# vilnik/incorporating-different-sources

Measured on AMD Instinct MI355X. Metric: rolling windows/sec, higher is better.
Workload: dtype f64

## Files before the change

### incorporating_different_sources_amd/csrc/posterior_wave_impl.h

```cpp
#pragma once
#include <utility>

#include "posterior_fused_impl.h"

namespace {

template <int NT_, bool LEAN_ = true>
struct WCfg {
    static constexpr int NT = NT_;
    static constexpr int KP = 16 * NT;
    static constexpr int NTILES = NT * (NT + 1) / 2;
    static constexpr int MLD = 17;
    static constexpr int OFF_M = 0;
    static constexpr int OFF_DG = OFF_M + NT * 16 * MLD;
    static constexpr int OFF_IDT = OFF_DG + 256;
    static constexpr int OFF_VEC = OFF_IDT + 256;
    static constexpr int LDS_DOUBLES = OFF_VEC + KP;
    static constexpr int LDS_BYTES = LDS_DOUBLES * 8;
    static constexpr int OFF_SUB = LDS_DOUBLES;
};
constexpr int WAVE_LDS_LIMIT = 64 * 1024;
__host__ __device__ inline int wave_idx_rows(int n_r, int m, bool conj) {
    const int r = (conj && m > n_r) ? m : n_r;
    return (r + 63) & ~63;
}
__host__ __device__ inline int wave_idx_bytes(int n_r, int m, bool conj) { return wave_idx_rows(n_r, m, conj) * 12; }

constexpr int wtile(int NT, int I, int J) { return I * NT - I * (I - 1) / 2 + (J - I); }

template <int I, int J>
__device__ __forceinline__ void wave_post_tile(double* P, int k, int fr, int fq, const d4& t) {
    const int gj = 16 * J + fr;
#pragma unroll
    for (int r = 0; r < 4; ++r) {
        const int gi = 16 * I + fq + 4 * r;
        if (gi < k && gj < k && (I < J || gi <= gj)) {
            tp_post_store(P + (long long)gi * k + gj, t[r]);
            if (I < J || gi < gj) tp_post_store(P + (long long)gj * k + gi, t[r]);
        }
    }
}

template <int NT, int NWV>
constexpr int w2_owner(int J) {
    const int p = NT - 1 - J, g = p / NWV, i = p % NWV;
    return (g & 1) ? NWV - 1 - i : i;
}
template <int NT, int NWV>
constexpr int w2_count(int WV) {
    int n = 0;
    for (int J = 0; J < NT; ++J)
        if (w2_owner<NT, NWV>(J) == WV) n += J + 1;
    return n;
}
template <int NT, int NWV>
constexpr int w2_max_tiles() {
    int m = 0;
    for (int w = 0; w < NWV; ++w) m = w2_count<NT, NWV>(w) > m ? w2_count<NT, NWV>(w) : m;
    return m;
}
template <int NT, int NWV>
constexpr int w2_slot(int I, int J) {
    const int wv = w2_owner<NT, NWV>(J);
    int n = 0;
    for (int i = 0; i < NT; ++i)
        for (int j = i; j < NT; ++j) {
            if (i == I && j == J) return n;
            if (w2_owner<NT, NWV>(j) == wv) ++n;
        }
    return -1;
}
template <int NT, int NWV>
constexpr bool w2_owns_from(int WV, int I) {
    for (int J = I; J < NT; ++J)
        if (w2_owner<NT, NWV>(J) == WV) return true;
    return false;
}
template <int NT>
constexpr bool w2_one_wave_is_whole() {
    for (int J = 0; J < NT; ++J) {
        if (w2_owner<NT, 1>(J) != 0) return false;
        for (int I = 0; I <= J; ++I)
            if (w2_slot<NT, 1>(I, J) != wtile(NT, I, J)) return false;
    }
    return w2_count<NT, 1>(0) == NT * (NT + 1) / 2;
}
template <int... N>
constexpr bool w2_one_wave_is_whole_all(std::integer_sequence<int, N...>) { return (w2_one_wave_is_whole<N + 1>() && ...); }
static_assert(w2_one_wave_is_whole_all(std::make_integer_sequence<int, 15>{}),
              "w2_owner<NT,1>(J) == 0, w2_slot<NT,1>(I,J) == wtile(NT,I,J), w2_count<NT,1>(0) == NT(NT+1)/2 for NT = 1..15");

constexpr bool wave_tile_in_agpr(int t) { return t < 32; }

template <int T>
__device__ __forceinline__ void wave_mfma_agpr(d4& c, double a, double b) {
    if constexpr (wave_tile_in_agpr(T)) asm volatile("s_nop 1\n\tv_mfma_f64_16x16x4_f64 %0, %1, %2, %0" : "+a"(c) : "v"(a), "v"(b));
    else asm volatile("s_nop 1\n\tv_mfma_f64_16x16x4_f64 %0, %1, %2, %0" : "+v"(c) : "v"(a), "v"(b));
}
template <int T>
__device__ __forceinline__ void wave_settle1(d4& c0) {
    if constexpr (wave_tile_in_agpr(T)) asm volatile("s_nop 15\n\ts_nop 7" : "+a"(c0));
    else asm volatile("s_nop 15\n\ts_nop 7" : "+v"(c0));
}
template <int T>
__device__ __forceinline__ void wave_pin1(d4& c0) {
    if constexpr (wave_tile_in_agpr(T)) asm volatile("" : "+a"(c0));
    else asm volatile("" : "+v"(c0));
}
__device__ __forceinline__ void wave_settle14(d4& c0, d4& c1, d4& c2, d4& c3, d4& c4, d4& c5, d4& c6, d4& c7, d4& c8, d4& c9,
                                              d4& c10, d4& c11, d4& c12, d4& c13) {
    asm volatile("s_nop 15\n\ts_nop 7" : "+a"(c0), "+a"(c1), "+a"(c2), "+a"(c3), "+a"(c4), "+a"(c5), "+a"(c6), "+a"(c7), "+a"(c8),
                 "+a"(c9), "+a"(c10), "+a"(c11), "+a"(c12), "+a"(c13));
}
template <int N>
__device__ __forceinline__ void wave_pin(d4 (&acc)[N]) {
    static_for<0, N>([&](auto tc) __attribute__((always_inline)) { wave_pin1<decltype(tc)::value>(acc[decltype(tc)::value]); });
}
template <bool GROUPED, int N>
__device__ __forceinline__ void wave_settle(d4 (&acc)[N]) {
    if constexpr (GROUPED) {
        static_for<0, (N + 13) / 14>([&](auto gc) __attribute__((always_inline)) {
            constexpr int b = 14 * decltype(gc)::value;
            if constexpr (b + 14 <= N && wave_tile_in_agpr(b + 13)) {
                wave_settle14(acc[b], acc[b + 1], acc[b + 2], acc[b + 3], acc[b + 4], acc[b + 5], acc[b + 6], acc[b + 7], acc[b + 8],
                              acc[b + 9], acc[b + 10], acc[b + 11], acc[b + 12], acc[b + 13]);
            } else {
                static_for<b, (b + 14 < N ? b + 14 : N)>([&](auto tc) __attribute__((always_inline)) {
                    wave_settle1<decltype(tc)::value>(acc[decltype(tc)::value]);
                });
            }
        });
    } else {
        wave_settle1<0>(acc[0]);
        static_for<1, N>([&](auto tc) __attribute__((always_inline)) { wave_pin1<decltype(tc)::value>(acc[decltype(tc)::value]); });
    }
}

struct WRows {
    const double* base;
    long long ld;
    const int* ridx;
    long long first;
    const double* sub_row;
    int count;
    int count0;
    int jump;
    bool off32 = false;
};

template <int NT, int NWV, int WV, bool HF, bool LEAN>
__device__ __forceinline__ void wave_gram(const WRows& src, const long long (&coff)[NT], int k, int lane,
                                          double (&shift)[NT], double (&w0v)[NT], bool ones, bool lazy_mask,
                                          d4 (&acc)[w2_count<NT, NWV>(WV)], const int* lds_rows, const double* lds_sub,
                                          double (&csum)[NT], double& usum) {
    constexpr int kI = NT - 1;
    const int fr = lane & 15, fq = lane >> 4;
    const int kc = k - 16 * kI;
    const bool cvl = fr < kc;
    const double border = HF ? ((ones && fr == kc + 1) ? 1.0 : 0.0) : ((fr == kc) ? 1.0 : 0.0);
    const int nks = (src.count + 3) >> 2;
    const bool has_sub = !HF && src.sub_row != nullptr;

    int row_pref = 0;
    double sub_pref = 0.0;
    auto prefetch = [&](int ks) __attribute__((always_inline)) {
        int r = 4 * ks + fq;
        r = r < src.count ? r : src.count - 1;
        row_pref = lds_rows[r];
        if (has_sub) sub_pref = lds_sub[r];
    };
    if constexpr (!LEAN) prefetch(0);
    const char* ub = (const char*)(LEAN ? src.base + src.first * src.ld : src.base);
    const unsigned ld8 = (unsigned)src.ld * 8u;
    unsigned c8[NT];
#pragma unroll
    for (int i = 0; i < NT; ++i) c8[i] = 8u * (unsigned)coff[i];
    auto load = [&](double (&v)[NT], double& sub, int ks) __attribute__((always_inline)) {
        int r = 4 * ks + fq;
        r = r < src.count ? r : src.count - 1;
        if (LEAN || src.off32) {
            unsigned row;
            if constexpr (LEAN) row = (unsigned)(r + (r >= src.count0 ? src.jump : 0));
            else row = (unsigned)row_pref;
            if constexpr (LEAN) {
                const unsigned r0 = __umul24(row, ld8) + c8[0];
#pragma unroll
                for (int i = 0; i < NT - 1; ++i) v[i] = *(const double*)(ub + (size_t)r0 + 128 * i);
                v[NT - 1] = *(const double*)(ub + (size_t)(__umul24(row, ld8) + c8[NT - 1]));
            } else {
                const unsigned ro = __umul24(row, ld8);
#pragma unroll
                for (int i = 0; i < NT; ++i) v[i] = *(const double*)(ub + (size_t)(ro + c8[i]));
            }
        } else {
            const double* p = src.base + (long long)row_pref * src.ld;
#pragma unroll
            for (int i = 0; i < NT; ++i) v[i] = p[coff[i]];
        }
        sub = 0.0;
        if constexpr (!LEAN) {
            if (has_sub) sub = sub_pref;
            prefetch(ks + 1);
        } else {
            if (has_sub) sub = src.sub_row[r];
        }
    };
    auto step = [&](double (&v)[NT], double sub, int ks, auto maskc) __attribute__((always_inline)) {
        constexpr bool MASK = decltype(maskc)::value != 0;
        if (HF) {
#pragma unroll
            for (int i = 0; i < NT; ++i) v[i] -= shift[i];
        } else if (has_sub) {
#pragma unroll
            for (int i = 0; i < NT; ++i) v[i] -= sub;
        }
        v[kI] = cvl ? v[kI] : border;
        if (MASK) {
            const bool rv = 4 * ks + fq < src.count;
#pragma unroll
            for (int i = 0; i < NT; ++i) v[i] = rv ? v[i] : 0.0;
        }
        if (HF) {
            double z = 0.0;
#pragma unroll
            for (int i = 0; i < NT; ++i) z = fma(v[i], w0v[i], z);
            z = rowgroup_sum16(z);
            if (!ones) {
#pragma unroll
                for (int i = 0; i < NT; ++i) csum[i] += v[i];
                usum += z;
            }
            if (fr == kc) v[kI] = z;
        }
        static_for<0, NT>([&](auto Ic) __attribute__((always_inline)) {
            constexpr int I = decltype(Ic)::value;
            static_for<I, NT>([&](auto Jc) __attribute__((always_inline)) {
                constexpr int J = decltype(Jc)::value;
                if constexpr (w2_owner<NT, NWV>(J) == WV) {
                    constexpr int t = w2_slot<NT, NWV>(I, J);
                    wave_mfma_agpr<t>(acc[t], v[I], v[J]);
                }
            });
        });
    };

    if (nks <= 0) return;
    double va[NT], vb[NT], vc[NT];
    double sa = 0.0, sb = 0.0, sc = 0.0;
    load(va, sa, 0);
    load(vb, sb, 1);
    if (HF && lazy_mask) {
        __builtin_amdgcn_sched_barrier(0);
#pragma unroll
        for (int i = 0; i < NT; ++i) {
            const bool cv = 16 * i + fr < k;
            shift[i] = cv ? shift[i] : 0.0;
            w0v[i] = cv ? w0v[i] : 0.0;
        }
    }
    wave_pin(acc);
    int ks = 0;
#pragma nounroll
    for (; 4 * (ks + 3) <= src.count; ks += 3) {
        load(vc, sc, ks + 2);
        step(va, sa, ks, ic<0>{});
        load(va, sa, ks + 3);
        step(vb, sb, ks + 1, ic<0>{});
        load(vb, sb, ks + 4);
        step(vc, sc, ks + 2, ic<0>{});
    }
    if (ks < nks) {
        if (ks + 2 < nks) load(vc, sc, ks + 2);
        step(va, sa, ks, ic<1>{});
        if (ks + 1 < nks) step(vb, sb, ks + 1, ic<1>{});
        if (ks + 2 < nks) step(vc, sc, ks + 2, ic<1>{});
    }
    wave_settle<NWV == 1>(acc);
}

__device__ __forceinline__ void wave_stage_rows(const WRows& src, int lane, int* li, double* lsb) {
    for (int i = lane; i < src.count; i += 64) {
        li[i] = src.ridx ? src.ridx[i] : (int)(src.first + i);
        if (src.sub_row) lsb[i] = src.sub_row[i];
    }
    __builtin_amdgcn_fence(__ATOMIC_RELEASE, "wavefront");
    __builtin_amdgcn_wave_barrier();
}

template <int NT, bool LEAN, int MODE>
__device__ __forceinline__ void wave_window_body(const tp_kargs_t& A, double* lds) {
    constexpr bool FULL = MODE == 2;
    constexpr bool POST = MODE >= 3;
    constexpr int PLAIN = POST ? MODE - 3 : MODE;
    using C = WCfg<NT, LEAN>;
    const int lane = threadIdx.x;
    const int fr = lane & 15, fq = lane >> 4;
    const int k = A.k;
    __builtin_assume(k >= 16 * (NT - 1));
    __builtin_assume(k <= 16 * NT - 1);
    constexpr int kI = NT - 1;
    const int kc = k - 16 * kI;
    const int NTB = (kc == 0) ? NT - 1 : NT;
    const bool colv = fr < kc;
    const long long per_xcd = (A.w_count + 7) >> 3;
    const long long wl = (long long)(blockIdx.x & 7) * per_xcd + (blockIdx.x >> 3);
    if ((long long)(blockIdx.x >> 3) >= per_xcd || wl >= A.w_count) return;
    const long long w = A.w_first + wl;
    const int tid0 = lane;
    (void)tid0;

    const int* cols = (!LEAN && A.col_idx) ? A.col_idx + w * k : nullptr;
    long long coff[NT];
    if (cols != nullptr) {
        int cidx[NT];
#pragma unroll
        for (int i = 0; i < NT; ++i) {
            const int c = 16 * i + fr;
            cidx[i] = cols[c < k ? c : k - 1];
        }
#pragma unroll
        for (int i = 0; i < NT; ++i) coff[i] = (long long)cidx[i];
    } else {
#pragma unroll
        for (int i = 0; i < NT; ++i) {
            const int c = 16 * i + fr;
            coff[i] = (long long)(c < k ? c : k - 1);
        }
    }
    double* idx_sub_lds = LEAN ? nullptr : lds + C::OFF_SUB;
    int* idx_rows_lds = LEAN ? nullptr : (int*)(lds + C::OFF_SUB + wave_idx_rows(A.n_r, A.m, A.strategy == 0));
    d4 acc[C::NTILES];
    static_for<0, C::NTILES>([&](auto tc) __attribute__((always_inline)) { acc[decltype(tc)::value] = d4{0.0, 0.0, 0.0, 0.0}; });
    wave_pin(acc);

#pragma unroll
    for (int i = 0; i < 4; ++i) {
        const int e = lane + 64 * i;
        lds[C::OFF_IDT + e] = ((e >> 4) == (e & 15)) ? 1.0 : 0.0;
    }

    double n0 = 0.0, cc = 0.0, q0 = 0.0;
    const bool conj = PLAIN == 0 ? true : PLAIN == 1 ? false : (A.strategy == 0);
    const int dbg = (FULL && A.dbg_S1 != nullptr && w == A.dbg_w) ? A.dbg_mode : 0;

    auto dump_matrix = [&]() __attribute__((always_inline)) {
        static_for<0, NT>([&](auto Ic) __attribute__((always_inline)) {
            constexpr int I = decltype(Ic)::value;
            static_for<I, NT>([&](auto Jc) __attribute__((always_inline)) {
                constexpr int J = decltype(Jc)::value;
                constexpr int t = wtile(NT, I, J);
                const int gj = 16 * J + fr;
#pragma unroll
                for (int r = 0; r < 4; ++r) {
                    const int gi = 16 * I + fq + 4 * r;
                    if (gi < k && gj < k) {
                        A.dbg_S1[(long long)gi * k + gj] = acc[t][r];
                        A.dbg_S1[(long long)gj * k + gi] = acc[t][r];
                    }
                    if (gi < k && gj == k) A.dbg_S1[(long long)k * k + gi] = acc[t][r];
                }
            });
        });
    };
    auto corner = [&]() __attribute__((always_inline)) {
        constexpr int t = wtile(NT, kI, kI);
        const int ln = __builtin_amdgcn_readfirstlane(16 * (kc & 3) + kc);
        const double x0 = readlane_d(acc[t][0], ln), x1 = readlane_d(acc[t][1], ln);
        const double x2 = readlane_d(acc[t][2], ln), x3 = readlane_d(acc[t][3], ln);
        const int rr = kc >> 2;
        return rr == 0 ? x0 : rr == 1 ? x1 : rr == 2 ? x2 : x3;
    };

    TP_MARK(0);
    if (conj && dbg != 2) {
        n0 = A.n0[w];
        WRows hs;
        hs.base = A.hf_panel; hs.ld = A.hf_ld;
        hs.ridx = (!LEAN && A.hf_row_idx) ? A.hf_row_idx + w * (long long)A.m : nullptr;
        hs.first = A.hf_start ? A.hf_start[w] : 0;
        hs.sub_row = nullptr;
        hs.count = A.hf_count ? A.hf_count[w] : A.m;
        hs.count0 = 0x7fffffff; hs.jump = 0;
        hs.off32 = (A.hf_off32 & 1) != 0;
        const bool ones = kc < 15;
        double shift[NT], w0v[NT], csum[NT];
        double usum = 0.0;
        {
            const long long row0 = hs.ridx ? (long long)hs.ridx[0] : hs.first;
            const double* p0 = hs.base + row0 * (long long)hs.ld;
#pragma unroll
            for (int i = 0; i < NT; ++i) {
                const int c = 16 * i + fr;
                const int cl = c < k ? c : k - 1;
                const double sv = p0[coff[i]];
                const double wv = A.w0[w * k + cl];
                shift[i] = sv;
                w0v[i] = wv;
                csum[i] = 0.0;
            }
        }
        TP_MARK(1);
        const int hf_rows_all = hs.count;
        if (!hs.ridx) { hs.first += 1; hs.count -= 1; }
        else { hs.ridx += 1; hs.count -= 1; }
        if constexpr (!LEAN) wave_stage_rows(hs, lane, idx_rows_lds, idx_sub_lds);
        wave_gram<NT, 1, 0, true, LEAN>(hs, coff, k, lane, shift, w0v, ones, true, acc, idx_rows_lds, idx_sub_lds, csum, usum);
        hs.count = hf_rows_all;
        TP_MARK(2);
        const double invm = 1.0 / (double)hs.count;
        double tj[NT];
        double cz = corner();
        if (ones) {
            static_for<0, NT>([&](auto Ic) __attribute__((always_inline)) {
                constexpr int I = decltype(Ic)::value;
                constexpr int t = wtile(NT, I, kI);
                if (fr == kc + 1) {
#pragma unroll
                    for (int r = 0; r < 4; ++r)
                        lds[C::OFF_VEC + 16 * I + fq + 4 * r] = (I < kI || fq + 4 * r <= kc) ? acc[t][r] : 0.0;
                }
            });
        } else {
#pragma unroll
            for (int i = 0; i < NT; ++i) {
                double sc_ = csum[i];
                sc_ += __shfl_xor(sc_, 16, 64);
                sc_ += __shfl_xor(sc_, 32, 64);
                if (fq == 0) lds[C::OFF_VEC + 16 * i + fr] = (16 * i + fr < k) ? sc_ : 0.0;
            }
            double su = usum;
            su += __shfl_xor(su, 16, 64);
            su += __shfl_xor(su, 32, 64);
            __builtin_amdgcn_fence(__ATOMIC_RELEASE, "wavefront");
            __builtin_amdgcn_wave_barrier();
            if (lane == 0) lds[C::OFF_VEC + k] = su;
        }
        __builtin_amdgcn_fence(__ATOMIC_RELEASE, "wavefront");
        __builtin_amdgcn_wave_barrier();
#pragma unroll
        for (int J = 0; J < NT; ++J) tj[J] = lds[C::OFF_VEC + 16 * J + fr];
        {
            const double tk = lds[C::OFF_VEC + k];
            cz = fma(-(tk * invm), tk, cz);
        }
        const double mm = (double)hs.count;
        const double sc = n0 * (mm / (mm - 1.0));
        q0 = sc * cz;
        const double a = n0 + k + 2;
        cc = (2 * n0) / (a + sqrt(a * a + 4 * n0 * q0));
        const double fcol = colv ? sc : ((fr == kc) ? cc * sc : 0.0);
        static_for<0, NT>([&](auto Ic) __attribute__((always_inline)) {
            constexpr int I = decltype(Ic)::value;
            double ti[4];
#pragma unroll
            for (int r = 0; r < 4; ++r) ti[r] = -(lds[C::OFF_VEC + 16 * I + fq + 4 * r] * invm);
            static_for<I, NT>([&](auto Jc) __attribute__((always_inline)) {
                constexpr int J = decltype(Jc)::value;
                constexpr int t = wtile(NT, I, J);
                d4 x = acc[t];
#pragma unroll
                for (int r = 0; r < 4; ++r) x[r] = fma(ti[r], tj[J], x[r]);
                if constexpr (J < kI) {
                    x *= sc;
                } else if constexpr (I < kI) {
                    x *= fcol;
                } else {
#pragma unroll
                    for (int r = 0; r < 4; ++r) x[r] *= (fq + 4 * r < kc) ? fcol : 0.0;
                }
                acc[t] = x;
                wave_pin1<t>(acc[t]);
            });
            __builtin_amdgcn_sched_barrier(0);
        });
        __builtin_amdgcn_wave_barrier();
        if (dbg == 1) { dump_matrix(); return; }
    }
    TP_MARK(3);
    {
        WRows ds;
        ds.base = A.panel; ds.ld = A.panel_ld;
        ds.ridx = (!LEAN && A.row_idx) ? A.row_idx + w * (long long)A.n_r : nullptr;
        ds.first = A.start ? A.start[w] : 0;
        ds.sub_row = A.rf_adj ? A.rf_adj + w * (long long)A.n_r : nullptr;
        ds.count = A.n_rows ? A.n_rows[w] : A.n_r;
        ds.count0 = 0x7fffffff; ds.jump = 0;
        ds.off32 = (A.panel_off32 & 1) != 0;
        double none[NT] = {};
        bool shared = false;
        const double* q = nullptr;
        if constexpr (LEAN) {
            constexpr int BLK = 16;
            const long long b0 = (ds.first + BLK - 1) / BLK, b1 = (ds.first + ds.count) / BLK;
            const int Lw = (int)(b1 - b0);
            const int li = Lw == A.winsum_L[0] ? 0 : Lw == A.winsum_L[1] ? 1 : Lw == A.winsum_L[2] ? 2 : Lw == A.winsum_L[3] ? 3 : -1;
            shared = A.winsum != nullptr && Lw > 0 && li >= 0;
            if (shared) {
                ds.count0 = (int)(BLK * b0 - ds.first);
                ds.jump = (int)(BLK * b1 - ds.first) - ds.count0;
                ds.count = ds.count0 + (int)(ds.first + ds.count - BLK * b1);
                q = A.winsum + ((long long)li * A.prefix_nblk + b0) * ((long long)C::NTILES * 256);
            }
        }
        TP_MARK(32);
        typedef double d2 __attribute__((ext_vector_type(2)));
        constexpr int GRP = 7, NG = (C::NTILES + GRP - 1) / GRP;
        const d2* pq = (const d2*)q + lane;
        d2 qa[GRP][2], qb[GRP][2];
        auto qload = [&](d2 (&v2)[GRP][2], auto gc) __attribute__((always_inline)) {
            constexpr int g = decltype(gc)::value;
            static_for<0, GRP>([&](auto ec) __attribute__((always_inline)) {
                constexpr int e = decltype(ec)::value;
                constexpr int t = g * GRP + e;
                if constexpr (t < C::NTILES) {
                    v2[e][0] = pq[(long long)t * 128];
                    v2[e][1] = pq[(long long)t * 128 + 64];
                }
            });
        };
        auto qadd = [&](d2 (&v2)[GRP][2], auto gc) __attribute__((always_inline)) {
            constexpr int g = decltype(gc)::value;
            static_for<0, GRP>([&](auto ec) __attribute__((always_inline)) {
                constexpr int e = decltype(ec)::value;
                constexpr int t = g * GRP + e;
                if constexpr (t < C::NTILES) {
                    d4 x = acc[t];
                    x[0] += v2[e][0][0]; x[1] += v2[e][0][1];
                    x[2] += v2[e][1][0]; x[3] += v2[e][1][1];
                    acc[t] = x;
                    wave_pin1<t>(acc[t]);
                }
            });
        };
        if constexpr (!LEAN) wave_stage_rows(ds, lane, idx_rows_lds, idx_sub_lds);
        double nosum = 0.0;
        wave_gram<NT, 1, 0, false, LEAN>(ds, coff, k, lane, none, none, false, false, acc, idx_rows_lds, idx_sub_lds, none, nosum);
        TP_MARK(33);
        if (LEAN && shared) {
            qload(qa, ic<0>{});
            static_for<0, NG>([&](auto gc) __attribute__((always_inline)) {
                constexpr int g = decltype(gc)::value;
                if constexpr (g + 1 < NG) {
                    if constexpr (g % 2 == 0) qload(qb, ic<g + 1>{}); else qload(qa, ic<g + 1>{});
                }
                __builtin_amdgcn_sched_barrier(0);
                if constexpr (g % 2 == 0) qadd(qa, gc); else qadd(qb, gc);
                __builtin_amdgcn_sched_barrier(0);
            });
        }
    }
    TP_MARK(34);
    static_for<0, NT>([&](auto Ic) __attribute__((always_inline)) {
        constexpr int I = decltype(Ic)::value;
        constexpr int t = wtile(NT, I, kI);
        if constexpr (I == kI) {
            d4 x = acc[t];
#pragma unroll
            for (int r = 0; r < 4; ++r) x[r] = (fq + 4 * r >= kc) ? 0.0 : x[r];
            acc[t] = x;
            wave_pin1<t>(acc[t]);
        }
    });
    __builtin_amdgcn_sched_barrier(0);
    if (dbg == 2) { dump_matrix(); return; }

    if (!conj) {
        static_for<0, NT>([&](auto Ic) __attribute__((always_inline)) {
            constexpr int I = decltype(Ic)::value;
            constexpr int t = wtile(NT, I, kI);
            if (fr == kc) {
#pragma unroll
                for (int r = 0; r < 4; ++r) lds[C::OFF_VEC + 16 * I + fq + 4 * r] = acc[t][r];
            }
        });
        __builtin_amdgcn_fence(__ATOMIC_RELEASE, "wavefront");
        __builtin_amdgcn_wave_barrier();
        const double invN = !FULL ? 1.0 / (double)A.N : A.center_rows == 2 ? 0.0
                          : 1.0 / (double)(A.center_rows ? (A.n_rows ? A.n_rows[w] : A.n_r) : A.N);
        const double sh_d = (FULL && A.shift) ? A.shift[2 * w] : 0.0;
        const double sh_e = (FULL && A.shift) ? A.shift[2 * w + 1] : 0.0;
        double tj[NT];
#pragma unroll
        for (int J = 0; J < NT; ++J) tj[J] = lds[C::OFF_VEC + 16 * J + fr];
        static_for<0, NT>([&](auto Ic) __attribute__((always_inline)) {
            constexpr int I = decltype(Ic)::value;
            double ti[4];
#pragma unroll
            for (int r = 0; r < 4; ++r) ti[r] = lds[C::OFF_VEC + 16 * I + fq + 4 * r];
            static_for<I, NT>([&](auto Jc) __attribute__((always_inline)) {
                constexpr int J = decltype(Jc)::value;
                constexpr int t = wtile(NT, I, J);
                d4 x = acc[t];
#pragma unroll
                for (int r = 0; r < 4; ++r) {
                    const bool on = (J < kI || colv) && (I < kI || fq + 4 * r < kc);
                    const double add = sh_e + ((I == J && fq + 4 * r == fr) ? sh_d : 0.0);
                    x[r] += on ? add - invN * (ti[r] * tj[J]) : 0.0;
                }
                acc[t] = x;
                wave_pin1<t>(acc[t]);
            });
            __builtin_amdgcn_sched_barrier(0);
        });
        __builtin_amdgcn_wave_barrier();
    }
    if (FULL && A.rhs != nullptr) {
        static_for<0, NT>([&](auto Ic) __attribute__((always_inline)) {
            constexpr int I = decltype(Ic)::value;
            constexpr int t = wtile(NT, I, kI);
            if (fr == kc) {
#pragma unroll
                for (int r = 0; r < 4; ++r) {
                    const int gi = 16 * I + fq + 4 * r;
                    const int gl = gi < k ? gi : k - 1;
                    const double x = A.rhs[w * k + gl];
                    acc[t][r] = (gi < k) ? x : 0.0;
                }
            }
            wave_pin1<t>(acc[t]);
        });
    }
    if (FULL && A.out_rhs != nullptr) {
        static_for<0, NT>([&](auto Ic) __attribute__((always_inline)) {
            constexpr int I = decltype(Ic)::value;
            constexpr int t = wtile(NT, I, kI);
            if (fr == kc) {
#pragma unroll
                for (int r = 0; r < 4; ++r) {
                    const int gi = 16 * I + fq + 4 * r;
                    if (gi < k) A.out_rhs[w * k + gi] = acc[t][r];
                }
            }
        });
    }
    if (dbg == 3) dump_matrix();
    if constexpr (POST) {
        double* P = tp_post_window(A, w);
        if (P != nullptr) {
            static_for<0, NT>([&](auto Ic) __attribute__((always_inline)) {
                constexpr int I = decltype(Ic)::value;
                static_for<I, NT>([&](auto Jc) __attribute__((always_inline)) {
                    constexpr int J = decltype(Jc)::value;
                    wave_post_tile<I, J>(P, k, fr, fq, acc[wtile(NT, I, J)]);
                });
            });
        }
    }

    TP_MARK(4);
    double badacc = 0.0;
    static_for<0, NT>([&](auto jc) __attribute__((always_inline)) {
        constexpr int j = decltype(jc)::value;
        if (j < NTB) {
            const int npiv = (k - 16 * j < 16) ? (k - 16 * j) : 16;
            constexpr int tjj = wtile(NT, j, j);
#pragma unroll
            for (int r = 0; r < 4; ++r) lds[C::OFF_DG + (fq + 4 * r) * 16 + fr] = acc[tjj][r];
            __builtin_amdgcn_fence(__ATOMIC_RELEASE, "wavefront");
            __builtin_amdgcn_wave_barrier();
            const int c16 = lane & 15;
            double a[16];
            const double* src = (lane < 16) ? (lds + C::OFF_DG) : (lds + C::OFF_IDT);
#pragma unroll
            for (int i = 0; i < 16; ++i) a[i] = src[i * 16 + c16];
            constexpr bool ALL16 = j < kI;
            double d0 = readlane_d(a[0], 0);
            double rinv = rsqrt_cubic(d0);
#pragma unroll
            for (int p = 0; p < 16; ++p) {
                if (ALL16 || p < npiv) {
                    a[p] *= rinv;
                    badacc = fma(0.0, rinv, badacc);
                    double rinv_next = 1.0;
                    if (p + 1 < 16) {
                        const double s1 = readlane_d(a[p], p + 1);
                        a[p + 1] = fma(-s1, a[p], a[p + 1]);
                        double dn = readlane_d(a[p + 1], p + 1);
                        if (!ALL16) dn = (p + 1 < npiv) ? dn : 1.0;
                        rinv_next = rsqrt_cubic(dn);
                    }
#pragma unroll
                    for (int i = p + 2; i < 16; ++i) {
                        const double sI = readlane_d(a[p], i);
                        a[i] = fma(-sI, a[p], a[i]);
                    }
                    rinv = rinv_next;
                    __builtin_amdgcn_sched_barrier(0);
                }
            }
            if (lane >= 16 && lane < 32) {
#pragma unroll
                for (int i = 0; i < 16; ++i) lds[C::OFF_M + (j * 16 + i) * C::MLD + c16] = (i < npiv) ? a[i] : 0.0;
            }
            __builtin_amdgcn_fence(__ATOMIC_RELEASE, "wavefront");
            __builtin_amdgcn_wave_barrier();
            double mop[4];
#pragma unroll
            for (int r = 0; r < 4; ++r) mop[r] = lds[C::OFF_M + (j * 16 + fr) * C::MLD + 4 * r + fq];
            static_for<j, NT>([&](auto Jc) __attribute__((always_inline)) {
                constexpr int J = decltype(Jc)::value;
                if constexpr (J > j || j == kI) {
                    constexpr int t = wtile(NT, j, J);
                    d4 rj = d4{0.0, 0.0, 0.0, 0.0};
#pragma unroll
                    for (int r = 0; r < 4; ++r) rj = __builtin_amdgcn_mfma_f64_16x16x4f64(mop[r], acc[t][r], rj, 0, 0, 0);
                    acc[t] = rj;
                }
            });
            static_for<j + 1, NT>([&](auto Ic) __attribute__((always_inline)) {
                constexpr int I = decltype(Ic)::value;
                static_for<I, NT>([&](auto Jc) __attribute__((always_inline)) {
                    constexpr int J = decltype(Jc)::value;
                    constexpr int t = wtile(NT, I, J), tI = wtile(NT, j, I), tJ = wtile(NT, j, J);
#pragma unroll
                    for (int r = 0; r < 4; ++r)
                        acc[t] = __builtin_amdgcn_mfma_f64_16x16x4f64(acc[tI][r], acc[tJ][r], acc[t], 0, 0, 1);
                });
            });
        }
    });

    TP_MARK(5);
    double q1 = 0.0;
    double wcol[NT];
#pragma unroll
    for (int J = 0; J < NT; ++J) wcol[J] = 0.0;
    {
        double q1p = 0.0;
        static_for<0, NT>([&](auto Ic) __attribute__((always_inline)) {
            constexpr int I = decltype(Ic)::value;
            constexpr int t = wtile(NT, I, kI);
#pragma unroll
            for (int r = 0; r < 4; ++r) {
                const double y = (fr == kc && (I < kI || fq + 4 * r < kc)) ? acc[t][r] : 0.0;
                q1p = fma(y, y, q1p);
            }
        });
        q1 = wave_sum64(q1p);
    }
    static_for<0, NT>([&](auto ic) __attribute__((always_inline)) {
        constexpr int Ib = NT - 1 - decltype(ic)::value;
        if (Ib < NTB) {
            constexpr int tb = wtile(NT, Ib, kI);
            double z[4];
#pragma unroll
            for (int r = 0; r < 4; ++r) {
                double u = 0.0;
                static_for<Ib + 1, NT>([&](auto Jc) __attribute__((always_inline)) {
                    constexpr int J = decltype(Jc)::value;
                    constexpr int t = wtile(NT, Ib, J);
                    if (J < NTB) u = fma(acc[t][r], wcol[J], u);
                });
                const double y = (fr == kc && (Ib < kI || fq + 4 * r < kc)) ? acc[tb][r] : 0.0;
                z[r] = rowgroup_sum16(y - u);
            }
            d4 wt = d4{0.0, 0.0, 0.0, 0.0};
#pragma unroll
            for (int r = 0; r < 4; ++r) {
                const double mrow = lds[C::OFF_M + (Ib * 16 + 4 * r + fq) * C::MLD + fr];
                wt = __builtin_amdgcn_mfma_f64_16x16x4f64(z[r], mrow, wt, 0, 0, 0);
            }
            wcol[Ib] = wt[0];
            __builtin_amdgcn_sched_barrier(0);
        }
    });

    TP_MARK(6);
    {
        const double n1 = n0 + (double)A.N;
        const double denom = n1 - q1;
        bool nonfinite = false;
        static_for<0, NT>([&](auto Ic) __attribute__((always_inline)) {
            constexpr int I = decltype(Ic)::value;
            const int gi = 16 * I + fr;
            double out;
            if (conj) out = 1.0 / A.gamma * ((n1 + k + 2) * wcol[I] / denom);
            else out = 1.0 / A.gamma * wcol[I];
            if (fq == (I & 3) && gi < k) {
                A.weights[w * k + gi] = out;
                if (!isfinite(out)) nonfinite = true;
            }
        });
        const bool anybad = __any(nonfinite ? 1 : 0) != 0;
        const bool notpd = __any((badacc != badacc) ? 1 : 0) != 0;
        if (lane == 0) {
            int st = TP_KSTATUS_OK;
            if (notpd) st = TP_KSTATUS_NOT_PD;
            else if (anybad) st = TP_KSTATUS_NONFINITE;
            else if (conj && !(denom > 0.0)) st = TP_KSTATUS_BAD_DENOM;
            A.status[w] = st;
            if (A.aux) {
                double* ax = A.aux + w * 8;
                ax[0] = n0; ax[1] = conj ? n1 : 0.0; ax[2] = cc; ax[3] = q0; ax[4] = q1;
                ax[5] = conj ? denom : 0.0; ax[6] = 0.0; ax[7] = 0.0;
            }
        }
    }
    TP_MARK(7);
}

constexpr int wave_occupancy(int nt) { return nt <= 3 ? 4 : nt <= 5 ? 2 : 1; }

template <int NT, bool LEAN, int MODE>
__global__ void __launch_bounds__(64, wave_occupancy(NT)) posterior_wave_kernel(const tp_kargs_t A) {
    extern __shared__ __attribute__((aligned(16))) double lds[];
    wave_window_body<NT, LEAN, MODE>(A, lds);
}

template <int NT, bool LEAN>
inline int wave_lds_bytes(const tp_kargs_t& a) {
    return WCfg<NT, LEAN>::LDS_BYTES + (LEAN ? 0 : wave_idx_bytes(a.n_r, a.m, a.strategy == 0));
}

constexpr bool wave_post_built(int nt, bool lean, int mode) { return !(mode == 3 && nt == 8 && !lean); }

template <int NT, bool LEAN, int MODE>
hipError_t wave_launch_mode(const tp_kargs_t& a, int grid8, hipStream_t stream) {
    if constexpr (!wave_post_built(NT, LEAN, MODE)) {
        return hipErrorNotSupported;
    } else {
        const int lds_bytes = wave_lds_bytes<NT, LEAN>(a);
        if (lds_bytes > WAVE_LDS_LIMIT) return hipErrorNotSupported;
        static std::atomic<unsigned long long> attr_done{0};
        { hipError_t e = tp_allow_dynamic_lds(attr_done, posterior_wave_kernel<NT, LEAN, MODE>, WAVE_LDS_LIMIT); if (e != hipSuccess) return e; }
        hipLaunchKernelGGL((posterior_wave_kernel<NT, LEAN, MODE>), dim3(grid8), dim3(64), lds_bytes, stream, a);
        return hipGetLastError();
    }
}

template <int NT, bool LEAN>
hipError_t wave_launch_variant(const tp_kargs_t& a, int grid, hipStream_t stream, tp_launch_info_t* info) {
    if (info) { info->grid = grid; info->block = 64; info->lds_bytes = wave_lds_bytes<NT, LEAN>(a); info->ntile = NT; }
    const int grid8 = 8 * ((grid + 7) / 8);
    const int mode = wave_mode(a);
    switch (mode == 2 ? 2 : tp_post_mode(a, mode)) {
        case 0: return wave_launch_mode<NT, LEAN, 0>(a, grid8, stream);
        case 1: return wave_launch_mode<NT, LEAN, 1>(a, grid8, stream);
        case 3: return wave_launch_mode<NT, LEAN, 3>(a, grid8, stream);
        case 4: return wave_launch_mode<NT, LEAN, 4>(a, grid8, stream);
        default: return hipErrorNotSupported;
    }
}

}
```

Baseline: 17.59 million.

## Broadcast Cholesky pivot row via LDS instead of per-element readlanes

In the in-wave 16x16 Cholesky panel factorization, the pivot row is written to LDS and read back with vectorized double2 loads for trailing rows beyond a small readlane window (RL=2). The diagonal update is computed lane-locally as a[p+1]-a[p]^2, and only the rsqrt result is read back with readlane. This cuts the many serialized v_readlane broadcasts per pivot step, but adds an LDS store, a wave barrier and LDS loads on each step's critical path. The reuse of the OFF_DG region as scratch and the lane mapping (lanes 16+ write to 32+lane) need to be correct.

Result: faster. 17.83 million, median of 6 (+1.4%).

```diff
diff --git a/incorporating_different_sources_amd/csrc/posterior_wave_impl.h b/incorporating_different_sources_amd/csrc/posterior_wave_impl.h
--- a/incorporating_different_sources_amd/csrc/posterior_wave_impl.h
+++ b/incorporating_different_sources_amd/csrc/posterior_wave_impl.h
@@ -664,6 +664,10 @@
 #pragma unroll
             for (int i = 0; i < 16; ++i) a[i] = src[i * 16 + c16];
             constexpr bool ALL16 = j < kI;
+            constexpr int RL = 2;
+            typedef double d2 __attribute__((ext_vector_type(2)));
+            double* const mrows = lds + C::OFF_DG;
+            const int mw = (lane < 16) ? lane : 32 + lane;
             double d0 = readlane_d(a[0], 0);
             double rinv = rsqrt_cubic(d0);
 #pragma unroll
@@ -671,19 +675,37 @@
                 if (ALL16 || p < npiv) {
                     a[p] *= rinv;
                     badacc = fma(0.0, rinv, badacc);
+                    const int i0 = p + 1 + RL;
+                    double* const mrow = mrows + 16 * (p & 1);
+                    if (i0 < 16) {
+                        mrow[mw] = a[p];
+                        __builtin_amdgcn_fence(__ATOMIC_RELEASE, "wavefront");
+                        __builtin_amdgcn_wave_barrier();
+                    }
+                    double mm[16];
+#pragma unroll
+                    for (int i = i0; i < 16; ++i) {
+                        if ((i & 1) == 0) {
+                            const d2 v = *(const d2*)(mrow + i);
+                            mm[i] = v[0];
+                            mm[i + 1] = v[1];
+                        } else if (i == i0) {
+                            mm[i] = mrow[i];
+                        }
+                    }
                     double rinv_next = 1.0;
                     if (p + 1 < 16) {
-                        const double s1 = readlane_d(a[p], p + 1);
-                        a[p + 1] = fma(-s1, a[p], a[p + 1]);
-                        double dn = readlane_d(a[p + 1], p + 1);
+                        double dn = fma(-a[p], a[p], a[p + 1]);
                         if (!ALL16) dn = (p + 1 < npiv) ? dn : 1.0;
-                        rinv_next = rsqrt_cubic(dn);
+                        rinv_next = readlane_d(rsqrt_cubic(dn), p + 1);
                     }
 #pragma unroll
-                    for (int i = p + 2; i < 16; ++i) {
+                    for (int i = p + 1; i < i0 && i < 16; ++i) {
                         const double sI = readlane_d(a[p], i);
                         a[i] = fma(-sI, a[p], a[i]);
                     }
+#pragma unroll
+                    for (int i = i0; i < 16; ++i) a[i] = fma(-mm[i], a[p], a[i]);
                     rinv = rinv_next;
                     __builtin_amdgcn_sched_barrier(0);
                 }
```
